# HDaoud/ORBSLAMM

Measured on AMD Instinct MI355X. Metric: frames/s ORB extract+match, 1241x376 @2000 kp; bit-exact kp/desc vs CPU, higher is better.
Workload: dtype u8

## Files before the change

### orbslamm_amd/csrc/orbx_host.inc

```

enum ProfId { P_H2D = 0, P_RESIZE, P_FAST, P_DISTRIBUTE, P_BLUR, P_ORIENT_DESC, P_MATCH_BEST2, P_MATCH_ACCEPT, P_MATCH_PRUNE, P_D2H, P_COUNT };
static const char* kProfNames[P_COUNT] = {"h2d", "k_pyramid", "k_fast", "k_distribute", "k_blur",
                                          "k_orient_desc", "k_match_mfma", "k_match_accept", "k_match_prune", "d2h"};
struct ProfSpan { int id; hipEvent_t a, b; };

struct Profiler {
    bool on = false, cur = false;
    int only = -1;
    std::vector<ProfSpan> spans;
    std::vector<hipEvent_t> pool;
    double ms[P_COUNT] = {0};
    int64_t launches[P_COUNT] = {0};
    hipEvent_t get()
    {
        if (!pool.empty()) { hipEvent_t e = pool.back(); pool.pop_back(); return e; }
        hipEvent_t e;
        (void)hipEventCreate(&e);
        return e;
    }
    void begin(int id, hipStream_t s)
    {
        cur = on && (only < 0 || only == id);
        if (!cur) return;
        ProfSpan sp{id, get(), get()};
// ... 305 lines not shown
    g.iniTh = h->prm.iniThFAST; g.minTh = h->prm.minThFAST;
    memcpy(g.umax, h->umax, sizeof g.umax);
    if (w > 8191 || h0 > 8191) return fail(ORBX_E_UNSUPPORTED, "frame larger than 8191 px");
    out.cells.clear();
    out.tabs.clear();
    int pyrOff = 0, blurOff = 0, candOff = 0, keptOff = 0, maxRoiW = 8, maxRoiH = 8, maxRoiW0 = 8, maxRoiH0 = 8, nodeCap = 16, maxCells = 1;
    for (int l = 0; l < g.nlevels; l++) {
        LevelGeom& L = g.lv[l];
        const float scale = h->mvInvScaleFactor[l];
        L.w = cv_round((double)((float)w * scale));
        L.h = cv_round((double)((float)h0 * scale));
        if (L.w < 1 || L.h < 1) return fail(ORBX_E_UNSUPPORTED, "pyramid level %d is empty", l);
        L.stride = align_up(L.w, 64);
        L.pyrOff = pyrOff;
        if (l > 0) pyrOff += align_up(L.stride * L.h, 256);
        L.blurStride = align_up(L.w, 64);
        L.blurOff = blurOff;
        blurOff += align_up(L.blurStride * L.h, 256);
        L.scale = h->mvScaleFactor[l];
        L.kpSize = (float)(int)((float)kPatchSize * h->mvScaleFactor[l]);
        L.nFeat = h->mnFeaturesPerLevel[l];

        const int minBX = kMinBorder, minBY = kMinBorder;
        const int maxBX = L.w - kEdgeThreshold + 3, maxBY = L.h - kEdgeThreshold + 3;
        L.winW = maxBX - minBX; L.winH = maxBY - minBY;
        const float W = 30;
        const float width = (float)(maxBX - minBX), height = (float)(maxBY - minBY);
        L.nCols = width > 0 ? (int)(width / W) : 0;
        L.nRows = height > 0 ? (int)(height / W) : 0;
        L.cellBase = (int)out.cells.size();
        L.nCells = 0;
        int candCap = 0;
        if (L.nCols >= 1 && L.nRows >= 1) {
            L.wCell = (int)std::ceil((double)(width / L.nCols));
            L.hCell = (int)std::ceil((double)(height / L.nRows));
            uint32_t seq = 0;
            for (int i = 0; i < L.nRows; i++) {
                const float iniY = (float)(minBY + i * L.hCell);
                float maxY = iniY + L.hCell + 6;
                if (iniY >= maxBY - 3) continue;
                if (maxY > maxBY) maxY = (float)maxBY;
                for (int j = 0; j < L.nCols; j++) {
                    const float iniX = (float)(minBX + j * L.wCell);
                    float maxX = iniX + L.wCell + 6;
                    if (iniX >= maxBX - 6) continue;
                    if (maxX > maxBX) maxX = (float)maxBX;
                    Cell c;
                    c.level = (uint16_t)l;
                    c.x0 = (uint16_t)(int)iniX; c.y0 = (uint16_t)(int)iniY;
                    c.w = (uint16_t)((int)maxX - (int)iniX); c.h = (uint16_t)((int)maxY - (int)iniY);
                    c.ci = (uint16_t)i; c.cj = (uint16_t)j;
                    c.seq = seq++;
                    c.candOff = (uint32_t)candCap;
                    if (c.w < 7 || c.h < 7) continue;
                    if (c.w > 127 || c.h > 127 || c.seq >= 65536u)
                        return fail(ORBX_E_UNSUPPORTED, "cell geometry out of range");
                    out.cells.push_back(c);
                    L.nCells++;
                    candCap += ((c.w - 6 + 1) / 2) * ((c.h - 6 + 1) / 2);
                    maxRoiW = std::max<int>(maxRoiW, c.w);
                    maxRoiH = std::max<int>(maxRoiH, c.h);
                    if (l == 0) { maxRoiW0 = std::max<int>(maxRoiW0, c.w); maxRoiH0 = std::max<int>(maxRoiH0, c.h); }
                }
            }
        }
        maxCells = std::max(maxCells, L.nCells);
        L.candOff = candOff;
        L.candCap = align_up(candCap + 8, 8);
        candOff += L.candCap;
        L.nIni = 0; L.hX = 0.f;
        if (L.winW > 0 && L.winH > 0) {
            L.nIni = (int)roundf((float)(maxBX - minBX) / (float)(maxBY - minBY));
            if (L.nIni >= 1) L.hX = (float)(maxBX - minBX) / (float)L.nIni;
            else if (L.nCells > 0)
                return fail(ORBX_E_UNSUPPORTED, "level %d: width/height < 0.5, the reference divides by zero (ORBextractor.cc:543-545)", l);
        }
        L.keptOff = keptOff;
        L.keptCap = align_up(std::max(L.nFeat + 4, 4 * L.nIni) + 4, 4);
        keptOff += L.keptCap;
        nodeCap = std::max(nodeCap, L.keptCap + 8);
    }
    g.totalCells = (int)out.cells.size();
    g.maxCellsPerLevel = maxCells;
    g.pyrFrameBytes = std::max(pyrOff, 256);
    g.blurFrameBytes = blurOff;
    g.candFrameRecs = candOff;
    g.keptFrameRecs = keptOff;
    g.maxKp = keptOff;
    out.tileStrideDw = maxRoiW + 5 <= 48 ? 12 : 20;
    if (maxRoiW + 5 > 80 || maxRoiW - 6 > 127 || maxRoiH - 6 > 127) return fail(ORBX_E_UNSUPPORTED, "cell larger than the FAST tile");
    out.tileRows = maxRoiH;
    out.fastListCap = ((maxRoiW - 6) * (maxRoiH - 6) + 63) / 64 * 64;
    out.tileRows0 = maxRoiH0;
    out.fastListCap0 = ((maxRoiW0 - 6) * (maxRoiH0 - 6) + 63) / 64 * 64;
    out.fastSmapPitch = align_up(maxRoiW - 6 + 2, 4);
    out.fastSmapPitch0 = align_up(maxRoiW0 - 6 + 2, 4);
    out.nodeCap = align_up(std::max(nodeCap, 360), 4);

    for (int l = 0; l < g.nlevels; l++) { out.xoff[l] = out.yoff[l] = 0; }
    for (int l = 1; l < g.nlevels; l++) {
        const int sw = g.lv[l - 1].w, sh = g.lv[l - 1].h, dw = g.lv[l].w, dh = g.lv[l].h;
        const double inv_scale_x = (double)dw / sw, inv_scale_y = (double)dh / sh;
        const double scale_x = 1. / inv_scale_x, scale_y = 1. / inv_scale_y;
        if (scale_x == 2.0 && scale_y == 2.0)
            return fail(ORBX_E_UNSUPPORTED, "scale factor 2: cv::resize switches to INTER_AREA (not on this path)");
        out.xoff[l] = (int)out.tabs.size();
        std::vector<short4> xt(dw);
        int xmax = dw;
        for (int dx = 0; dx < dw; dx++) {
            float fx = (float)((dx + 0.5) * scale_x - 0.5);
            int sx = (int)std::floor(fx);
            fx -= sx;
            if (sx < 0) { fx = 0; sx = 0; }
            if (sx + 1 >= sw) {
                xmax = std::min(xmax, dx);
                if (sx >= sw - 1) { fx = 0; sx = sw - 1; }
            }
            auto sat = [](float v) { long r = lrintf(v); return (short)(r > 32767 ? 32767 : (r < -32768 ? -32768 : r)); };
            xt[dx] = make_short4((short)sx, sat((1.f - fx) * 2048), sat(fx * 2048), 0);
        }
        for (int dx = 0; dx < dw; dx++) xt[dx].w = dx < xmax ? 1 : 0;
        out.tabs.insert(out.tabs.end(), xt.begin(), xt.end());
        out.yoff[l] = (int)out.tabs.size();
        for (int dy = 0; dy < dh; dy++) {
            float fy = (float)((dy + 0.5) * scale_y - 0.5);
            int sy = (int)std::floor(fy);
            fy -= sy;
            auto clip = [&](int y) { return y < 0 ? 0 : (y < sh ? y : sh - 1); };
            auto sat = [](float v) { long r = lrintf(v); return (short)(r > 32767 ? 32767 : (r < -32768 ? -32768 : r)); };
            out.tabs.push_back(make_short4((short)clip(sy), (short)clip(sy + 1), sat((1.f - fy) * 2048), sat(fy * 2048)));
        }
    }
    int tb = 0, kb = 0;
    for (int l = 0; l < g.nlevels; l++) {
        out.bt.base[l] = tb;
        out.bt.tilesX[l] = (g.lv[l].w + kBlurTW - 1) / kBlurTW;
        tb += out.bt.tilesX[l] * ((g.lv[l].h + kBlurTH - 1) / kBlurTH);
        out.kb.base[l] = kb;
        kb += (g.lv[l].keptCap + kKpPerBlock - 1) / kKpPerBlock;
    }
    for (int l = g.nlevels; l <= ORBX_MAXL; l++) { out.bt.base[l] = tb; out.kb.base[l] = kb; }
    out.blurTilesTotal = tb;
    out.kbTotal = kb;

    out.pyrFused = false;
    const int refine0 = h->maxB <= h->latMaxB ? 1 : 0;
    for (int refine = refine0; refine < 4 && !out.pyrFused; refine++) {
        const int nl = g.nlevels;
        const int top = nl - 1;
        int BX = 4 << refine, BY = 6 << refine;
        while (BX > 1 && g.lv[top].w / BX < 8) BX >>= 1;
        while (BY > 1 && g.lv[top].h / BY < 8) BY >>= 1;
        out.pyrBlocks = BX * BY;
        out.pyrRanges.assign((size_t)out.pyrBlocks * nl, PyrRange{0, 0, 0, 0, 0, 0, 0, 0});
        int maxA = 4, maxB = 4, tabCap = 4;
        for (int bj = 0; bj < BY; bj++)
            for (int bi = 0; bi < BX; bi++) {
                PyrRange* R = &out.pyrRanges[(size_t)(bj * BX + bi) * nl];
                int nx0 = 0, nx1 = 0, ny0 = 0, ny1 = 0;
                for (int l = top; l >= 0; l--) {
                    const int w = g.lv[l].w, hh = g.lv[l].h;
                    int ox0 = (int)((int64_t)bi * w / BX) & ~3, ox1 = bi + 1 == BX ? w : ((int)((int64_t)(bi + 1) * w / BX) & ~3);
                    int oy0 = (int)((int64_t)bj * hh / BY), oy1 = (int)((int64_t)(bj + 1) * hh / BY);
                    if (l == 0) ox0 = ox1 = oy0 = oy1 = 0;
                    int cx0 = ox0, cx1 = ox1, cy0 = oy0, cy1 = oy1;
                    if (l < top && nx1 > nx0 && ny1 > ny0) {
                        const short4* xt = &out.tabs[out.xoff[l + 1]];
                        const short4* yt = &out.tabs[out.yoff[l + 1]];
                        int sx0 = 1 << 30, sx1 = -1, sy0 = 1 << 30, sy1 = -1;
                        const int nx1g = std::min<int>(g.lv[l + 1].w, nx0 + ((nx1 - nx0 + 3) & ~3));
                        for (int dx = nx0; dx < nx1g; dx++) {
                            const int a = (uint16_t)xt[dx].x, b = a + (xt[dx].w ? 2 : 1);
                            sx0 = std::min(sx0, a); sx1 = std::max(sx1, b);
                        }
                        for (int dy = ny0; dy < ny1; dy++) {
                            sy0 = std::min<int>(sy0, yt[dy].x); sy1 = std::max<int>(sy1, yt[dy].y + 1);
                        }
                        sx1 = std::min(sx1, w); sy1 = std::min(sy1, hh);
                        if (cx1 > cx0 && cy1 > cy0) {
                            cx0 = std::min(cx0, sx0); cx1 = std::max(cx1, sx1);
                            cy0 = std::min(cy0, sy0); cy1 = std::max(cy1, sy1);
                        } else { cx0 = sx0; cx1 = sx1; cy0 = sy0; cy1 = sy1; }
                    }
                    cx0 &= ~3;
                    R[l] = PyrRange{(int16_t)ox0, (int16_t)ox1, (int16_t)oy0, (int16_t)oy1,
                                    (int16_t)cx0, (int16_t)cx1, (int16_t)cy0, (int16_t)cy1};
                    if (cx1 > cx0 && cy1 > cy0) {
                        const int rowBytes = (cx1 - cx0 + 3) & ~3;
                        int rows = cy1 - cy0;
                        if (l == 0 && ny1 > ny0) {
                            const short4* yt = &out.tabs[out.yoff[1]];
                            const int chh1 = ny1 - ny0;
                            rows = 0;
                            for (int sidx = 0; sidx < kPyrStrips; sidx++) {
                                const int ya = (int)((int64_t)chh1 * sidx / kPyrStrips), yb = (int)((int64_t)chh1 * (sidx + 1) / kPyrStrips);
                                if (yb > ya) rows = std::max(rows, std::min<int>(yt[ny0 + yb - 1].y + 1, cy1) - (int)yt[ny0 + ya].x);
                            }
                        }
                        const int words = rowBytes / 4 * rows + 4;
                        if (l & 1) maxB = std::max(maxB, words); else maxA = std::max(maxA, words);
                        if (l > 0) tabCap = std::max(tabCap, std::max(rowBytes, cy1 - cy0));
                    }
                    nx0 = cx0; nx1 = cx1; ny0 = cy0; ny1 = cy1;
                }
            }
        out.pyrBufA = maxA; out.pyrBufB = maxB; out.pyrTabCap = (tabCap + 3) & ~3;
        const size_t pl = ((size_t)maxA + maxB) * 4 + (size_t)out.pyrTabCap * 16;
        out.pyrFused = pl <= 64 * 1024 || (refine == 3 && pl <= 156 * 1024);
    }
    return ORBX_OK;
}

static constexpr int kMatchChunks = 4;

static size_t dist_lds_bytes(int cap, int maxCells) { return (size_t)(19 * cap + 8 + 2 * (maxCells + 1)) * 4; }

static void chain_stream_release(int device, int idx);
static void tput_streams_release(orbx_handle* h);

static void free_device(orbx_handle* h)
{
    if (h->device < 0) return;
    (void)hipSetDevice(h->device);
    if (h->stream) (void)hipStreamSynchronize(h->stream);
    for (int i = 0; i < orbx_handle::kMaxSplit; i++) {
        if (h->streamP[i]) (void)hipStreamSynchronize(h->streamP[i]);
        if (h->streamB[i]) (void)hipStreamSynchronize(h->streamB[i]);
    }
    if (h->stream3) (void)hipStreamSynchronize(h->stream3);
    h->prof.destroy();
    void* ptrs[] = {h->d_distScratch, h->d_pyrRanges, h->d_geom, h->d_cells, h->d_tabs, h->d_pyr, h->d_blur, h->d_candRaw, h->d_candA, h->d_candB,
                    h->d_candCount, h->d_cellCount, h->d_kept, h->d_keptCount, h->d_err, h->d_kps, h->d_desc, h->d_count,
                    h->d_match, h->d_binOf, h->d_hist, h->d_nmatch, h->d_partial, h->d_xdesc};
    for (void* p : ptrs) if (p) (void)hipFree(p);
    if (h->d_stereo) (void)hipFree(h->d_stereo);
    h->pool.stop();
    for (hipStream_t st : {h->streamUp, h->streamDown, h->streamUpQ, h->streamDownQ}) if (st) (void)hipStreamSynchronize(st);
    for (auto& sl : h->slot) {
        if (sl.h_in) (void)hipHostFree(sl.h_in);
        if (sl.h_out) (void)hipHostFree(sl.h_out);
        if (sl.d_in) (void)hipFree(sl.d_in);
        if (sl.d_out) (void)hipFree(sl.d_out);
        for (hipEvent_t& e : sl.evUp) if (e) (void)hipEventDestroy(e);
        if (sl.evOut) (void)hipEventDestroy(sl.evOut);
        if (sl.evPacked) (void)hipEventDestroy(sl.evPacked);
    }
    for (hipStream_t st : {h->streamUp, h->streamDown, h->streamUpQ, h->streamDownQ}) if (st) (void)hipStreamDestroy(st);
    for (int i = 0; i < orbx_handle::kMaxSplit; i++) {
        if (h->evPyr[i]) (void)hipEventDestroy(h->evPyr[i]);
        if (h->evBlur[i]) (void)hipEventDestroy(h->evBlur[i]);
        if (h->evPart[i]) (void)hipEventDestroy(h->evPart[i]);
        if (h->evFast0[i]) (void)hipEventDestroy(h->evFast0[i]);
        if (h->streamP[i] && !(i == 0 && h->chainIdx >= 0) && !h->sharedStreams) (void)hipStreamDestroy(h->streamP[i]);
        if (h->streamB[i]) (void)hipStreamDestroy(h->streamB[i]);
    }
    if (h->evStart) (void)hipEventDestroy(h->evStart);
    if (h->evDesc) (void)hipEventDestroy(h->evDesc);
    for (int i = 0; i < 2; i++) if (h->evMatch[i]) (void)hipEventDestroy(h->evMatch[i]);
    for (int i = 0; i < 2; i++) if (h->evMatched[i]) (void)hipEventDestroy(h->evMatched[i]);
    if (h->sharedStreams) tput_streams_release(h);
    if (h->stream3) (void)hipStreamDestroy(h->stream3);
    if (h->stream) (void)hipStreamDestroy(h->stream);
    if (h->chainIdx >= 0) { chain_stream_release(h->device, h->chainIdx); h->chainIdx = -1; h->streamP[0] = nullptr; }
}

struct ChainPool { hipStream_t s[4] = {nullptr, nullptr, nullptr, nullptr}; int users[4] = {0, 0, 0, 0}; bool made = false; };
static ChainPool g_chain[64];
static std::mutex g_chainMu;

static bool chain_prio_normal() { static const bool v = [] { const char* e = getenv("ORBX_LAT_PRIO"); return e && e[0] == '0'; }(); return v; }

static int chain_stream_acquire(int device, int priority, hipStream_t* out, int* idx)
{
    std::lock_guard<std::mutex> lk(g_chainMu);
    ChainPool& cp = g_chain[device & 63];
    if (!cp.made) {
        hipStream_t s[4] = {nullptr, nullptr, nullptr, nullptr};
        void* scratch = nullptr;
        hipError_t e = hipMalloc(&scratch, 256);
        for (int i = 0; i < 4 && e == hipSuccess; i++) e = hipStreamCreateWithPriority(&s[i], hipStreamNonBlocking, priority);
        for (int i = 0; i < 4 && e == hipSuccess; i++) { e = hipMemsetAsync(scratch, 0, 256, s[i]); if (e == hipSuccess) e = hipStreamSynchronize(s[i]); }
        if (scratch) (void)hipFree(scratch);
        if (e != hipSuccess) {
            for (hipStream_t st : s) if (st) (void)hipStreamDestroy(st);
            return fail(ORBX_E_HIP, "cannot make the chain streams of device %d: %s", device, hipGetErrorString(e));
        }
        for (int i = 0; i < 4; i++) cp.s[i] = s[i];
        cp.made = true;
    }
    int best = 0;
    for (int i = 1; i < 4; i++) if (cp.users[i] < cp.users[best]) best = i;
    cp.users[best]++;
    *out = cp.s[best]; *idx = best;
    return ORBX_OK;
}

static void chain_stream_release(int device, int idx)
{
    std::lock_guard<std::mutex> lk(g_chainMu);
    if (idx >= 0 && idx < 4) g_chain[device & 63].users[idx]--;
}

struct TputPool { hipStream_t host = nullptr, p[orbx_handle::kMaxSplit] = {nullptr}, match = nullptr; int users = 0; };
static TputPool g_tput[64];
static std::mutex g_tputMu;

static int tput_streams_acquire(orbx_handle* h, int device, int prHi)
{
    std::lock_guard<std::mutex> lk(g_tputMu);
    TputPool& tp = g_tput[device & 63];
    if (!tp.host) {
        TputPool t;
        void* scratch = nullptr;
        hipError_t e = hipStreamCreateWithFlags(&t.host, hipStreamNonBlocking);
        if (e == hipSuccess) e = hipStreamCreateWithPriority(&t.p[0], hipStreamNonBlocking, prHi);
        if (e == hipSuccess) e = hipStreamCreateWithPriority(&t.p[1], hipStreamNonBlocking, prHi);
        if (e == hipSuccess) e = hipStreamCreateWithFlags(&t.match, hipStreamNonBlocking);
        if (e == hipSuccess) e = hipMalloc(&scratch, 256);
        for (hipStream_t st : {t.host, t.p[0], t.p[1], t.match}) {
            if (e == hipSuccess) e = hipMemsetAsync(scratch, 0, 256, st);
            if (e == hipSuccess) e = hipStreamSynchronize(st);
        }
        if (scratch) (void)hipFree(scratch);
        for (int i = 2; i < orbx_handle::kMaxSplit && e == hipSuccess; i++) e = hipStreamCreateWithPriority(&t.p[i], hipStreamNonBlocking, prHi);
        if (e != hipSuccess) {
            for (hipStream_t st : {t.host, t.match}) if (st) (void)hipStreamDestroy(st);
            for (hipStream_t st : t.p) if (st) (void)hipStreamDestroy(st);
            return fail(ORBX_E_HIP, "cannot make the pipeline streams of device %d: %s", device, hipGetErrorString(e));
        }
        tp.host = t.host; tp.match = t.match;
        for (int i = 0; i < orbx_handle::kMaxSplit; i++) tp.p[i] = t.p[i];
    }
    tp.users++;
    h->stream = tp.host; h->stream3 = tp.match;
    for (int i = 0; i < orbx_handle::kMaxSplit; i++) h->streamP[i] = tp.p[i];
    h->sharedStreams = true;
    return ORBX_OK;
}

static void tput_streams_release(orbx_handle* h)
{
    std::lock_guard<std::mutex> lk(g_tputMu);
    TputPool& tp = g_tput[h->device & 63];
    h->stream = nullptr; h->stream3 = nullptr;
    for (int i = 0; i < orbx_handle::kMaxSplit; i++) h->streamP[i] = nullptr;
    h->sharedStreams = false;
    --tp.users;
}

static int create_handle(const OrbxParams* params, int max_w, int max_h, int max_batch, int device, int latCeil, orbx_t** out)
{
    if (!params || !out) return fail(ORBX_E_INVALID, "null argument");
    *out = nullptr;
    orbx_handle* h = new orbx_handle();
    h->latMaxB = latCeil;
    h->prm = *params;
    int rc = init_tables(h);
    if (rc) { delete h; return rc; }
    h->device = device;
    { const char* e = getenv("ORBX_SERIAL"); h->serial = e && e[0] == '1'; }
    { const char* e = getenv("ORBX_MATCH_POPCOUNT"); h->matchPopcount = e && e[0] == '1'; }
// ... 1359 lines not shown
```

### orbslamm_amd/csrc/orbx_kernels.hip

```cpp
#include <hip/hip_runtime.h>
#include <stdint.h>

#include "orbx_common.hpp"

namespace orbx {

struct FrameSrc {
    const uint8_t* img0;
    int32_t stride0;
    int64_t pitch0;
    uint8_t* pyr;
    uint8_t* blur;
    int32_t f0;
};

__device__ __forceinline__ const uint8_t* level_ptr(const Geom* g, const FrameSrc& s, int f, int l, int& stride)
{
    if (l == 0) { stride = s.stride0; return s.img0 + (int64_t)f * s.pitch0; }
    stride = g->lv[l].stride;
    return s.pyr + (int64_t)f * g->pyrFrameBytes + g->lv[l].pyrOff;
}

__device__ __forceinline__ bool xcd_block_frame(int nframes, int& blk, int& fr)
{
    if (nframes < 8) { blk = blockIdx.x; fr = blockIdx.y; return true; }
    const int total = gridDim.x;
    const int lin = blockIdx.y * total + blockIdx.x;
    const int k = lin >> 3;
    fr = (k / total) * 8 + (lin & 7);
    blk = k - (k / total) * total;
    return fr < nframes;
}

__device__ __forceinline__ uint64_t lanemask_lt()
{
    const uint32_t lane = threadIdx.x & 63;
    return lane == 0 ? 0ull : (~0ull >> (64 - lane));
}

struct ResizeTabs {
    const short4* xtab[ORBX_MAXL];
    const short4* ytab[ORBX_MAXL];
};

__global__ __launch_bounds__(256) void k_resize_level(const Geom* __restrict__ g, FrameSrc src, ResizeTabs tabs, int level)
{
    const int lw = g->lv[level].w, lh = g->lv[level].h, dstStride = g->lv[level].stride;
    const int f = blockIdx.z + src.f0;
    const int x4 = (blockIdx.x * 64 + threadIdx.x) * 4;
    const int dy = blockIdx.y * 4 + threadIdx.y;
    if (x4 >= lw || dy >= lh) return;
    int sstride;
    const uint8_t* S = level_ptr(g, src, f, level - 1, sstride);
    uint8_t* D = src.pyr + (int64_t)f * g->pyrFrameBytes + g->lv[level].pyrOff + (int64_t)dy * dstStride;
    const short4 yt = tabs.ytab[level][dy];
    const uint8_t* S0 = S + (int64_t)yt.x * sstride;
    const uint8_t* S1 = S + (int64_t)yt.y * sstride;
    const int b0 = yt.z, b1 = yt.w;
    uint32_t packed = 0;
#pragma unroll
    for (int i = 0; i < 4; i++) {
        const short4 xt = tabs.xtab[level][min(x4 + i, lw - 1)];
        const int sx = (uint16_t)xt.x;
        int r0, r1;
        if (xt.w) {
            r0 = S0[sx] * xt.y + S0[sx + 1] * xt.z;
            r1 = S1[sx] * xt.y + S1[sx + 1] * xt.z;
        } else {
            r0 = S0[sx] * 2048;
            r1 = S1[sx] * 2048;
        }
        const int v = (((b0 * (r0 >> 4)) >> 16) + ((b1 * (r1 >> 4)) >> 16) + 2) >> 2;
        packed |= (uint32_t)(v & 0xFF) << (8 * i);
    }
    *(uint32_t*)(D + x4) = packed;
}

constexpr int kPyrStrips = 2;
#ifndef ORBX_DESC_PRIO
#define ORBX_DESC_PRIO 0
#endif
#ifndef ORBX_BLUR_PRIO
#define ORBX_BLUR_PRIO 0
#endif
#ifndef ORBX_DIST_PRIO
#define ORBX_DIST_PRIO 0
#endif
#ifndef ORBX_PYR_PRIO
#define ORBX_PYR_PRIO 3
#endif
#ifndef ORBX_PYR_THREADS
#define ORBX_PYR_THREADS 256
#endif
constexpr int kPyrThreads = ORBX_PYR_THREADS;
struct PyrRange {
    int16_t ox0, ox1, oy0, oy1;
    int16_t nx0, nx1, ny0, ny1;
};

__global__ __launch_bounds__(kPyrThreads) void k_pyramid(const Geom* __restrict__ g, FrameSrc src, ResizeTabs tabs,
                                                const PyrRange* __restrict__ ranges, int bufAWords, int bufBWords,
                                                int tabCap, int xcdFrames)
{
    extern __shared__ __attribute__((aligned(16))) uint32_t plds[];
#if ORBX_PYR_PRIO
    __builtin_amdgcn_s_setprio(ORBX_PYR_PRIO);
#endif
    uint8_t* const ldsb = (uint8_t*)plds;
    const int offBuf[2] = {0, bufAWords * 4};
    uint2* const sxt = (uint2*)(plds + bufAWords + bufBWords);
    uint2* const syt = sxt + tabCap;
    int pblk = (int)blockIdx.x, pfr = (int)blockIdx.y;
    if (xcdFrames >= 8 && !xcd_block_frame(xcdFrames, pblk, pfr)) return;
    const int f = pfr + src.f0;
    const int nl = g->nlevels;
    const PyrRange* R = ranges + (int64_t)pblk * nl;
    const int tid = threadIdx.x;

    PyrRange p = R[0];
    int pstride = 0;
    const bool have0 = p.nx1 > p.nx0 && p.ny1 > p.ny0;
    int stride0 = 0;
    const uint8_t* S0 = nullptr;
    int ndw0 = 0;
    if (have0) {
        const uint8_t* S = level_ptr(g, src, f, 0, stride0);
        ndw0 = (p.nx1 - p.nx0 + 3) >> 2;
        pstride = ndw0 * 4;
        S0 = S + p.nx0;
    }
    constexpr int T = kPyrThreads;
    constexpr int kStripRegs = 4096 / T;
    uint32_t sreg[kStripRegs];
    auto strip_rows = [&](int strip, int chh1, const uint2* yt, int& r0, int& r1) {
        const int ya = (int)((int64_t)chh1 * strip / kPyrStrips), yb = (int)((int64_t)chh1 * (strip + 1) / kPyrStrips);
        r0 = r1 = 0;
        if (yb > ya) { r0 = (int16_t)(yt[ya].x & 0xFFFF); r1 = min((int)(int16_t)(yt[yb - 1].x >> 16) + 1, (int)p.ny1); }
    };
    const int q256 = have0 ? T / ndw0 : 0, m256 = have0 ? T - q256 * ndw0 : 0;
    const int rowT = have0 ? tid / ndw0 : 0, colT = have0 ? tid - rowT * ndw0 : 0;
    auto fetch0 = [&](int r0, int r1) {
        const int total = (r1 - r0) * ndw0;
        if (total <= 0 || total > T * kStripRegs) return;
        const uint8_t* Sr = S0 + (int64_t)r0 * stride0;
        int r = rowT, c = colT;
#pragma unroll
        for (int k = 0; k < kStripRegs; k++) {
            if (k * T < total) {
                if (k * T + tid < total) sreg[k] = *(const uint32_t*)(Sr + (int64_t)r * stride0 + 4 * c);
                r += q256; c += m256;
                if (c >= ndw0) { c -= ndw0; r++; }
            }
        }
    };
    auto commit0 = [&](int r0, int r1) {
        const int total = (r1 - r0) * ndw0;
        if (total <= 0) return;
        if (total <= T * kStripRegs) {
#pragma unroll
            for (int k = 0; k < kStripRegs; k++) {
                const int i = k * T + tid;
                if (i < total) plds[i] = sreg[k];
            }
            return;
        }
        const uint8_t* Sr = S0 + (int64_t)r0 * stride0;
        for (int i0 = 0; i0 < total; i0 += T * 8) {
            uint32_t regs[8];
#pragma unroll
            for (int k = 0; k < 8; k++) {
                const int i = min(i0 + k * T + tid, total - 1);
                const int r = i / ndw0, c = i - r * ndw0;
                regs[k] = *(const uint32_t*)(Sr + (int64_t)r * stride0 + 4 * c);
            }
#pragma unroll
            for (int k = 0; k < 8; k++) {
                const int i = i0 + k * T + tid;
                if (i < total) plds[i] = regs[k];
            }
        }
    };
    for (int l = 1; l < nl; l++) {
        const PyrRange c = R[l];
        const int cw = c.nx1 - c.nx0, chh = c.ny1 - c.ny0;
        const int gpr = (cw + 3) >> 2;
        const int cstride = gpr * 4;
        const int lw = g->lv[l].w, dstStride = g->lv[l].stride;
        uint8_t* const D = src.pyr + (int64_t)f * g->pyrFrameBytes + g->lv[l].pyrOff;
        const int pnx0 = p.nx0, pny0 = p.ny0;
        const uint2* __restrict__ gx_tab = (const uint2*)tabs.xtab[l];
        const uint2* __restrict__ gy_tab = (const uint2*)tabs.ytab[l];
        for (int i = tid; i < cstride; i += T) sxt[i] = gx_tab[min(c.nx0 + i, lw - 1)];
        for (int i = tid; i < chh; i += T) syt[i] = gy_tab[c.ny0 + i];
        __syncthreads();
        const int offP = offBuf[(l - 1) & 1], offC = offBuf[l & 1];
        const bool strips = l == 1 && have0 && chh > 0;
        const int nstrips = strips ? kPyrStrips : 1;
        if (strips) { int r0, r1; strip_rows(0, chh, syt, r0, r1); fetch0(r0, r1); }
        for (int strip = 0; strip < nstrips; strip++) {
        const int ya = strips ? (int)((int64_t)chh * strip / nstrips) : 0, yb = strips ? (int)((int64_t)chh * (strip + 1) / nstrips) : chh;
        int prow0 = pny0;
        if (strips) {
            int r0, r1;
            strip_rows(strip, chh, syt, r0, r1);
            prow0 = r0;
            if (strip) __syncthreads();
            commit0(r0, r1);
            __syncthreads();
            if (strip + 1 < nstrips) { int q0, q1; strip_rows(strip + 1, chh, syt, q0, q1); fetch0(q0, q1); }
        }
        if (gpr > 0 && yb > ya) {
          for (int gxb = 0; gxb < gpr; gxb += T) {
            const int cols = min(T, gpr - gxb);
            const int dr = T / cols;
            const int yy0 = tid / cols, gx = gxb + tid - yy0 * cols;
            if (yy0 < dr) {
                int sx[4], a0[4], a1[4];
#pragma unroll
                for (int i = 0; i < 4; i++) {
                    const uint2 xt = sxt[4 * gx + i];
                    sx[i] = (int)(xt.x & 0xFFFF) - pnx0;
                    a0[i] = (int16_t)(xt.x >> 16);
                    a1[i] = (int16_t)(xt.y & 0xFFFF);
                }
                const int dx = c.nx0 + 4 * gx;
                const bool ownX = dx >= c.ox0 && dx < c.ox1;
                for (int yy = ya + yy0; yy < yb; yy += dr) {
                    const uint2 yt = syt[yy];
                    const int sy0 = (int16_t)(yt.x & 0xFFFF), sy1 = (int16_t)(yt.x >> 16);
                    const int b0 = (int16_t)(yt.y & 0xFFFF), b1 = (int16_t)(yt.y >> 16);
                    const int o0 = offP + (sy0 - prow0) * pstride;
                    const int o1 = offP + (sy1 - prow0) * pstride;
                    uint32_t packed = 0;
#pragma unroll
                    for (int i = 0; i < 4; i++) {
                        const int s00 = ldsb[o0 + sx[i]], s10 = ldsb[o1 + sx[i]];
                        const int r0 = s00 * a0[i] + ldsb[o0 + sx[i] + 1] * a1[i];
                        const int r1 = s10 * a0[i] + ldsb[o1 + sx[i] + 1] * a1[i];
                        const int v = (((b0 * (r0 >> 4)) >> 16) + ((b1 * (r1 >> 4)) >> 16) + 2) >> 2;
                        packed |= (uint32_t)(v & 0xFF) << (8 * i);
                    }
                    plds[(offC >> 2) + yy * gpr + gx] = packed;
                    const int dy = c.ny0 + yy;
                    if (ownX && dy >= c.oy0 && dy < c.oy1)
                        *(uint32_t*)(D + (int64_t)dy * dstStride + dx) = packed;
                }
            }
          }
        }
        }
        p = c;
        pstride = cstride;
        __syncthreads();
    }
}

__device__ __forceinline__ int min3i(int a, int b, int c) { return min(min(a, b), c); }
__device__ __forceinline__ int max3i(int a, int b, int c) { return max(max(a, b), c); }

template <int TSB, int K> struct RingOff {
    static constexpr int cx[16] = {0, 1, 2, 3, 3, 3, 2, 1, 0, -1, -2, -3, -3, -3, -2, -1};
    static constexpr int cy[16] = {3, 3, 2, 1, 0, -1, -2, -3, -3, -3, -2, -1, 0, 1, 2, 3};
    static constexpr int v = cx[K] + cy[K] * TSB;
};

__device__ __forceinline__ int arc_max_of_min(const int (&d)[16])
{
    int m3[16], m9[16];
#pragma unroll
    for (int k = 0; k < 16; k++) m3[k] = min3i(d[k], d[(k + 1) & 15], d[(k + 2) & 15]);
#pragma unroll
    for (int k = 0; k < 16; k++) m9[k] = min3i(m3[k], m3[(k + 3) & 15], m3[(k + 6) & 15]);
    int a5[5];
#pragma unroll
    for (int k = 0; k < 5; k++) a5[k] = max3i(m9[3 * k], m9[3 * k + 1], m9[3 * k + 2]);
    return max(max3i(a5[0], a5[1], a5[2]), max3i(a5[3], a5[4], m9[15]));
}

template <int TSB> __device__ __forceinline__ void ring_load(const uint8_t* __restrict__ p, int (&r)[16])
{
    r[0] = p[RingOff<TSB, 0>::v];   r[1] = p[RingOff<TSB, 1>::v];   r[2] = p[RingOff<TSB, 2>::v];   r[3] = p[RingOff<TSB, 3>::v];
    r[4] = p[RingOff<TSB, 4>::v];   r[5] = p[RingOff<TSB, 5>::v];   r[6] = p[RingOff<TSB, 6>::v];   r[7] = p[RingOff<TSB, 7>::v];
    r[8] = p[RingOff<TSB, 8>::v];   r[9] = p[RingOff<TSB, 9>::v];   r[10] = p[RingOff<TSB, 10>::v]; r[11] = p[RingOff<TSB, 11>::v];
    r[12] = p[RingOff<TSB, 12>::v]; r[13] = p[RingOff<TSB, 13>::v]; r[14] = p[RingOff<TSB, 14>::v]; r[15] = p[RingOff<TSB, 15>::v];
}

template <int SW> __device__ __forceinline__ uint32_t pk_min3(uint32_t a, uint32_t b, uint32_t c)
{
    uint32_t r;
    if (SW == 0) asm("v_pk_minimum3_f16 %0, %1, %2, %3" : "=v"(r) : "v"(a), "v"(b), "v"(c));
    else if (SW == 4) asm("v_pk_minimum3_f16 %0, %1, %2, %3 op_sel:[0,0,1] op_sel_hi:[1,1,0]" : "=v"(r) : "v"(a), "v"(b), "v"(c));
    else if (SW == 6) asm("v_pk_minimum3_f16 %0, %1, %2, %3 op_sel:[0,1,1] op_sel_hi:[1,0,0]" : "=v"(r) : "v"(a), "v"(b), "v"(c));
    else asm("v_pk_minimum3_f16 %0, %1, %2, %3 op_sel:[0,1,0] op_sel_hi:[1,0,1]" : "=v"(r) : "v"(a), "v"(b), "v"(c));
    static_assert(SW == 0 || SW == 2 || SW == 4 || SW == 6, "exchange masks in use");
    return r;
}
template <int SW> __device__ __forceinline__ uint32_t pk_max3(uint32_t a, uint32_t b, uint32_t c)
{
    uint32_t r;
    if (SW == 0) asm("v_pk_maximum3_f16 %0, %1, %2, %3" : "=v"(r) : "v"(a), "v"(b), "v"(c));
    else if (SW == 4) asm("v_pk_maximum3_f16 %0, %1, %2, %3 op_sel:[0,0,1] op_sel_hi:[1,1,0]" : "=v"(r) : "v"(a), "v"(b), "v"(c));
    else if (SW == 6) asm("v_pk_maximum3_f16 %0, %1, %2, %3 op_sel:[0,1,1] op_sel_hi:[1,0,0]" : "=v"(r) : "v"(a), "v"(b), "v"(c));
    else asm("v_pk_maximum3_f16 %0, %1, %2, %3 op_sel:[0,1,0] op_sel_hi:[1,0,1]" : "=v"(r) : "v"(a), "v"(b), "v"(c));
    static_assert(SW == 0 || SW == 2 || SW == 4 || SW == 6, "exchange masks in use");
    return r;
}
template <bool MAXMIN> __device__ __forceinline__ int arc_fold_pk(const int (&r)[16])
{
    uint32_t X[8], M3[8], M9[8];
#pragma unroll
    for (int k = 0; k < 8; k++) X[k] = (uint32_t)r[k] | ((uint32_t)r[k + 8] << 16);
#define ORBX_IN(SW, a, b, c) (MAXMIN ? pk_min3<SW>(a, b, c) : pk_max3<SW>(a, b, c))
#define ORBX_OUT(SW, a, b, c) (MAXMIN ? pk_max3<SW>(a, b, c) : pk_min3<SW>(a, b, c))
#pragma unroll
    for (int k = 0; k < 6; k++) M3[k] = ORBX_IN(0, X[k], X[k + 1], X[k + 2]);
    M3[6] = ORBX_IN(4, X[6], X[7], X[0]);
    M3[7] = ORBX_IN(6, X[7], X[0], X[1]);
    M9[0] = ORBX_IN(0, M3[0], M3[3], M3[6]);
    M9[1] = ORBX_IN(0, M3[1], M3[4], M3[7]);
    M9[2] = ORBX_IN(4, M3[2], M3[5], M3[0]);
    M9[3] = ORBX_IN(4, M3[3], M3[6], M3[1]);
    M9[4] = ORBX_IN(4, M3[4], M3[7], M3[2]);
    M9[5] = ORBX_IN(6, M3[5], M3[0], M3[3]);
    M9[6] = ORBX_IN(6, M3[6], M3[1], M3[4]);
    M9[7] = ORBX_IN(6, M3[7], M3[2], M3[5]);
    const uint32_t A = ORBX_OUT(0, M9[0], M9[1], M9[2]);
    const uint32_t B = ORBX_OUT(0, M9[3], M9[4], M9[5]);
    const uint32_t C = ORBX_OUT(0, M9[6], M9[7], A);
    const uint32_t D = ORBX_OUT(4, B, C, B);
    const uint32_t E = ORBX_OUT(2, D, C, D);
#undef ORBX_IN
#undef ORBX_OUT
    return (int)(E & 0xFFFFu);
}

template <int TSB> __device__ __forceinline__ int fast_S_dark(const uint8_t* __restrict__ p)
{
    int r[16];
    ring_load<TSB>(p, r);
    return max((int)p[0] - arc_fold_pk<false>(r), 0);
}
template <int TSB> __device__ __forceinline__ int fast_S_bright(const uint8_t* __restrict__ p)
{
    int r[16];
    ring_load<TSB>(p, r);
    return max(arc_fold_pk<true>(r) - (int)p[0], 0);
}

template <int TSB> __device__ __forceinline__ int fast_S(const uint8_t* __restrict__ p)
{
    int r[16], d[16];
    ring_load<TSB>(p, r);
    const int v = p[0];
#pragma unroll
    for (int k = 0; k < 16; k++) d[k] = v - r[k];
    const int A = arc_max_of_min(d);
#pragma unroll
    for (int k = 0; k < 16; k++) d[k] = -d[k];
    return max(max(A, arc_max_of_min(d)), 0);
}

__device__ __forceinline__ uint64_t ballot64(bool b) { return __builtin_amdgcn_ballot_w64(b); }
__device__ __forceinline__ uint64_t tail_mask(int n) { return n >= 64 ? ~0ull : (1ull << n) - 1; }
__device__ __forceinline__ int lanes_below(uint64_t bal)
{
    return __builtin_amdgcn_mbcnt_hi((uint32_t)(bal >> 32), __builtin_amdgcn_mbcnt_lo((uint32_t)bal, 0));
}

#ifdef ORBX_FAST_STATS
__device__ unsigned long long g_fastStats[16];
#endif
template <int TSB>
__global__ __launch_bounds__(64) void k_fast(const Geom* __restrict__ g, const Cell* __restrict__ cells,
                                            FrameSrc src, uint64_t* __restrict__ cand,
                                            int32_t* __restrict__ cellCount, int32_t* __restrict__ errFlag,
                                            int tileRows, int listCap, int smapPitch, int nframes, int cell0)
{
    extern __shared__ __attribute__((aligned(16))) uint32_t lds[];
    constexpr int TSD = TSB / 4;
    int bx, fr;
    if (!xcd_block_frame(nframes, bx, fr)) return;
    bx += cell0;
    const Cell c = cells[bx];
    const int f = fr + src.f0;
    const int lane = threadIdx.x;
    const int level = c.level;
    const LevelGeom& L = g->lv[level];
    int stride;
    const uint8_t* base = level_ptr(g, src, f, level, stride);

#ifdef ORBX_FAST_STATS
    unsigned long long tk0 = wall_clock64(), tk1;
    const bool statCell = lane == 0 && (blockIdx.x & 63) == 0;
#define FAST_TICK(i) do { tk1 = wall_clock64(); if (statCell) atomicAdd(&g_fastStats[i], tk1 - tk0); tk0 = tk1; } while (0)
#else
#define FAST_TICK(i) do { } while (0)
#endif
    uint32_t* tile = lds;
// ... 1493 lines not shown
```

Measured before the change: 184,100.

## Tune pyramid resize inner loop: precomputed LDS offsets, chunk widths, packed rounding

The y-table now stores row offsets relative to the previous-level LDS buffer, computed once per strip, so the inner loop does not recompute them per output row. The host picks a per-strip column chunk width that minimises wavefront-iterations, replacing the fixed width of T. Ownership tests move to a single unsigned range compare with incrementally stepped pointers. Rounding and packing use SDWA inline assembly plus v_perm. The fused-pyramid condition also gains a per-buffer size cap. This adds ISA-specific asm and a bigger PyrRange struct, and bit-exactness depends on the packed adds never overflowing their 16-bit halves.

```diff
diff --git a/orbslamm_amd/csrc/orbx_host.inc b/orbslamm_amd/csrc/orbx_host.inc
--- a/orbslamm_amd/csrc/orbx_host.inc
+++ b/orbslamm_amd/csrc/orbx_host.inc
@@ -481,7 +481,7 @@
         while (BX > 1 && g.lv[top].w / BX < 8) BX >>= 1;
         while (BY > 1 && g.lv[top].h / BY < 8) BY >>= 1;
         out.pyrBlocks = BX * BY;
-        out.pyrRanges.assign((size_t)out.pyrBlocks * nl, PyrRange{0, 0, 0, 0, 0, 0, 0, 0});
+        out.pyrRanges.assign((size_t)out.pyrBlocks * nl, PyrRange{0, 0, 0, 0, 0, 0, 0, 0, {}});
         int maxA = 4, maxB = 4, tabCap = 4;
         for (int bj = 0; bj < BY; bj++)
             for (int bi = 0; bi < BX; bi++) {
@@ -513,7 +513,14 @@
                     }
                     cx0 &= ~3;
                     R[l] = PyrRange{(int16_t)ox0, (int16_t)ox1, (int16_t)oy0, (int16_t)oy1,
-                                    (int16_t)cx0, (int16_t)cx1, (int16_t)cy0, (int16_t)cy1};
+                                    (int16_t)cx0, (int16_t)cx1, (int16_t)cy0, (int16_t)cy1, {}};
+                    if (l > 0 && cx1 > cx0 && cy1 > cy0) {
+                        const int gpr = (cx1 - cx0 + 3) >> 2, rows = cy1 - cy0;
+                        for (int sidx = 0; sidx < kPyrStrips; sidx++) {
+                            const int ya = (int)((int64_t)rows * sidx / kPyrStrips), yb = (int)((int64_t)rows * (sidx + 1) / kPyrStrips);
+                            R[l].cw[sidx] = (int16_t)pyr_chunk_width(gpr, l == 1 ? yb - ya : rows, kPyrThreads);
+                        }
+                    }
                     if (cx1 > cx0 && cy1 > cy0) {
                         const int rowBytes = (cx1 - cx0 + 3) & ~3;
                         int rows = cy1 - cy0;
@@ -535,7 +542,7 @@
             }
         out.pyrBufA = maxA; out.pyrBufB = maxB; out.pyrTabCap = (tabCap + 3) & ~3;
         const size_t pl = ((size_t)maxA + maxB) * 4 + (size_t)out.pyrTabCap * 16;
-        out.pyrFused = pl <= 64 * 1024 || (refine == 3 && pl <= 156 * 1024);
+        out.pyrFused = pl <= 64 * 1024 || (refine == 3 && pl <= 156 * 1024 && std::max(maxA, maxB) <= 16 * 1024);
     }
     return ORBX_OK;
 }
diff --git a/orbslamm_amd/csrc/orbx_kernels.hip b/orbslamm_amd/csrc/orbx_kernels.hip
--- a/orbslamm_amd/csrc/orbx_kernels.hip
+++ b/orbslamm_amd/csrc/orbx_kernels.hip
@@ -93,10 +93,41 @@
 #define ORBX_PYR_THREADS 256
 #endif
 constexpr int kPyrThreads = ORBX_PYR_THREADS;
-struct PyrRange {
+struct alignas(4) PyrRange {
     int16_t ox0, ox1, oy0, oy1;
     int16_t nx0, nx1, ny0, ny1;
+    int16_t cw[kPyrStrips];
 };
+
+static inline int pyr_chunk_cost(int gpr, int rows, int c, int T)
+{
+    int cost = 0;
+    for (int g0 = 0; g0 < gpr; g0 += c) {
+        const int cols = gpr - g0 < c ? gpr - g0 : c, dr = T / cols;
+        cost += (cols * dr + 63) / 64 * ((rows + dr - 1) / dr);
+    }
+    return cost;
+}
+static inline int pyr_chunk_width(int gpr, int rows, int T)
+{
+    if (gpr <= 0 || rows <= 0) return 1;
+    int best = gpr < T ? gpr : T, bestCost = pyr_chunk_cost(gpr, rows, best, T);
+    for (int c = best - 1; c >= 1; c--) {
+        const int cost = pyr_chunk_cost(gpr, rows, c, T);
+        if (cost < bestCost) { best = c; bestCost = cost; }
+    }
+    return best;
+}
+
+__device__ __forceinline__ uint32_t pyr_round_pack(uint32_t sum0, uint32_t q01, uint32_t q11, uint32_t sum2, uint32_t q03, uint32_t q13)
+{
+    asm("v_add_u32_sdwa %0, %2, %3 dst_sel:WORD_1 dst_unused:UNUSED_PRESERVE src0_sel:WORD_1 src1_sel:WORD_1\n\t"
+        "v_add_u32_sdwa %1, %4, %5 dst_sel:WORD_1 dst_unused:UNUSED_PRESERVE src0_sel:WORD_1 src1_sel:WORD_1\n\t"
+        "v_add_u32_e32 %0, 0x20002, %0\n\t"
+        "v_add_u32_e32 %1, 0x20002, %1"
+        : "+v"(sum0), "+v"(sum2) : "v"(q01), "v"(q11), "v"(q03), "v"(q13));
+    return __builtin_amdgcn_perm(sum2 >> 2, sum0 >> 2, 0x06040200u);
+}
 
 __global__ __launch_bounds__(kPyrThreads) void k_pyramid(const Geom* __restrict__ g, FrameSrc src, ResizeTabs tabs,
                                                 const PyrRange* __restrict__ ranges, int bufAWords, int bufBWords,
@@ -132,10 +163,10 @@
     constexpr int T = kPyrThreads;
     constexpr int kStripRegs = 4096 / T;
     uint32_t sreg[kStripRegs];
-    auto strip_rows = [&](int strip, int chh1, const uint2* yt, int& r0, int& r1) {
+    auto strip_rows = [&](int strip, int chh1, const short4* __restrict__ yt, int& r0, int& r1) {
         const int ya = (int)((int64_t)chh1 * strip / kPyrStrips), yb = (int)((int64_t)chh1 * (strip + 1) / kPyrStrips);
         r0 = r1 = 0;
-        if (yb > ya) { r0 = (int16_t)(yt[ya].x & 0xFFFF); r1 = min((int)(int16_t)(yt[yb - 1].x >> 16) + 1, (int)p.ny1); }
+        if (yb > ya) { r0 = yt[ya].x; r1 = min((int)yt[yb - 1].y + 1, (int)p.ny1); }
     };
     const int q256 = have0 ? T / ndw0 : 0, m256 = have0 ? T - q256 * ndw0 : 0;
     const int rowT = have0 ? tid / ndw0 : 0, colT = have0 ? tid - rowT * ndw0 : 0;
@@ -189,61 +220,86 @@
         uint8_t* const D = src.pyr + (int64_t)f * g->pyrFrameBytes + g->lv[l].pyrOff;
         const int pnx0 = p.nx0, pny0 = p.ny0;
         const uint2* __restrict__ gx_tab = (const uint2*)tabs.xtab[l];
-        const uint2* __restrict__ gy_tab = (const uint2*)tabs.ytab[l];
+        const uint2* __restrict__ gy_tab = (const uint2*)tabs.ytab[l] + c.ny0;
+        const short4* __restrict__ gy_rows = tabs.ytab[l] + c.ny0;
+        const bool strips = l == 1 && have0 && chh > 0;
+        const int nstrips = strips ? kPyrStrips : 1;
+        int srow0[kPyrStrips];
+#pragma unroll
+        for (int s = 0; s < kPyrStrips; s++) {
+            srow0[s] = pny0;
+            if (strips) { int r1; strip_rows(s, chh, gy_rows, srow0[s], r1); }
+        }
+        if (strips) { int r0, r1; strip_rows(0, chh, gy_rows, r0, r1); fetch0(r0, r1); }
         for (int i = tid; i < cstride; i += T) sxt[i] = gx_tab[min(c.nx0 + i, lw - 1)];
-        for (int i = tid; i < chh; i += T) syt[i] = gy_tab[c.ny0 + i];
+        for (int i = tid; i < chh; i += T) {
+            const uint2 yt = gy_tab[i];
+            int prow = srow0[0];
+#pragma unroll
+            for (int s = 1; s < kPyrStrips; s++)
+                if (strips && i >= (int)((int64_t)chh * s / kPyrStrips)) prow = srow0[s];
+            const uint32_t o0 = (uint32_t)(((int)(int16_t)(yt.x & 0xFFFF) - prow) * pstride);
+            const uint32_t o1 = (uint32_t)(((int)(int16_t)(yt.x >> 16) - prow) * pstride);
+            syt[i] = make_uint2((o0 & 0xFFFF) | (o1 << 16), yt.y);
+        }
         __syncthreads();
         const int offP = offBuf[(l - 1) & 1], offC = offBuf[l & 1];
-        const bool strips = l == 1 && have0 && chh > 0;
-        const int nstrips = strips ? kPyrStrips : 1;
-        if (strips) { int r0, r1; strip_rows(0, chh, syt, r0, r1); fetch0(r0, r1); }
         for (int strip = 0; strip < nstrips; strip++) {
         const int ya = strips ? (int)((int64_t)chh * strip / nstrips) : 0, yb = strips ? (int)((int64_t)chh * (strip + 1) / nstrips) : chh;
-        int prow0 = pny0;
         if (strips) {
             int r0, r1;
-            strip_rows(strip, chh, syt, r0, r1);
-            prow0 = r0;
+            strip_rows(strip, chh, gy_rows, r0, r1);
             if (strip) __syncthreads();
             commit0(r0, r1);
             __syncthreads();
-            if (strip + 1 < nstrips) { int q0, q1; strip_rows(strip + 1, chh, syt, q0, q1); fetch0(q0, q1); }
+            if (strip + 1 < nstrips) { int q0, q1; strip_rows(strip + 1, chh, gy_rows, q0, q1); fetch0(q0, q1); }
         }
         if (gpr > 0 && yb > ya) {
-          for (int gxb = 0; gxb < gpr; gxb += T) {
-            const int cols = min(T, gpr - gxb);
+          int C = c.cw[0];
+#pragma unroll
+          for (int s = 1; s < kPyrStrips; s++) if (strip == s) C = c.cw[s];
+          C = min(max(C, 1), T);
+          for (int gxb = 0; gxb < gpr; gxb += C) {
+            const int cols = min(C, gpr - gxb);
             const int dr = T / cols;
             const int yy0 = tid / cols, gx = gxb + tid - yy0 * cols;
             if (yy0 < dr) {
-                int sx[4], a0[4], a1[4];
+                uint32_t sxo[4], a0[4], a1[4];
 #pragma unroll
                 for (int i = 0; i < 4; i++) {
                     const uint2 xt = sxt[4 * gx + i];
-                    sx[i] = (int)(xt.x & 0xFFFF) - pnx0;
-                    a0[i] = (int16_t)(xt.x >> 16);
-                    a1[i] = (int16_t)(xt.y & 0xFFFF);
+                    sxo[i] = (uint32_t)(offP + (int)(xt.x & 0xFFFF) - pnx0);
+                    a0[i] = xt.x >> 16;
+                    a1[i] = xt.y & 0xFFFF;
                 }
                 const int dx = c.nx0 + 4 * gx;
                 const bool ownX = dx >= c.ox0 && dx < c.ox1;
-                for (int yy = ya + yy0; yy < yb; yy += dr) {
-                    const uint2 yt = syt[yy];
-                    const int sy0 = (int16_t)(yt.x & 0xFFFF), sy1 = (int16_t)(yt.x >> 16);
-                    const int b0 = (int16_t)(yt.y & 0xFFFF), b1 = (int16_t)(yt.y >> 16);
-                    const int o0 = offP + (sy0 - prow0) * pstride;
-                    const int o1 = offP + (sy1 - prow0) * pstride;
-                    uint32_t packed = 0;
+                const int ownA = ownX ? min(max(ya, c.oy0 - c.ny0), yb) : yb;
+                const int ownB = ownX ? max(ownA, min(yb, c.oy1 - c.ny0)) : yb;
+                const uint32_t nOwn = (uint32_t)(ownB - ownA);
+                const int tEnd = yb - ownA;
+                const int y0 = ya + yy0;
+                const uint2* yp = syt + y0;
+                uint32_t* outp = plds + (offC >> 2) + y0 * gpr + gx;
+                uint32_t goff = (uint32_t)((c.ny0 + y0) * dstStride + dx);
+                const uint32_t gstep = (uint32_t)(dr * dstStride);
+                for (int t = y0 - ownA; t < tEnd; t += dr, yp += dr, outp += dr * gpr, goff += gstep) {
+                    const uint2 yt = *yp;
+                    const uint32_t o0 = yt.x & 0xFFFF, o1 = yt.x >> 16;
+                    const uint32_t b0 = yt.y & 0xFFFF, b1 = yt.y >> 16;
+                    uint32_t q0[4], q1[4];
 #pragma unroll
                     for (int i = 0; i < 4; i++) {
-                        const int s00 = ldsb[o0 + sx[i]], s10 = ldsb[o1 + sx[i]];
-                        const int r0 = s00 * a0[i] + ldsb[o0 + sx[i] + 1] * a1[i];
-                        const int r1 = s10 * a0[i] + ldsb[o1 + sx[i] + 1] * a1[i];
-                        const int v = (((b0 * (r0 >> 4)) >> 16) + ((b1 * (r1 >> 4)) >> 16) + 2) >> 2;
-                        packed |= (uint32_t)(v & 0xFF) << (8 * i);
+                        const uint32_t p0 = sxo[i] + o0, p1 = sxo[i] + o1;
+                        const uint32_t s00 = ldsb[p0], s10 = ldsb[p1];
+                        const uint32_t r0 = s00 * a0[i] + ldsb[p0 + 1] * a1[i];
+                        const uint32_t r1 = s10 * a0[i] + ldsb[p1 + 1] * a1[i];
+                        q0[i] = b0 * (r0 >> 4);
+                        q1[i] = b1 * (r1 >> 4);
                     }
-                    plds[(offC >> 2) + yy * gpr + gx] = packed;
-                    const int dy = c.ny0 + yy;
-                    if (ownX && dy >= c.oy0 && dy < c.oy1)
-                        *(uint32_t*)(D + (int64_t)dy * dstStride + dx) = packed;
+                    const uint32_t packed = pyr_round_pack((q0[0] >> 16) + (q1[0] >> 16), q0[1], q1[1], (q0[2] >> 16) + (q1[2] >> 16), q0[3], q1[3]);
+                    *outp = packed;
+                    if ((uint32_t)t < nOwn) *(uint32_t*)(D + goff) = packed;
                 }
             }
           }
```

New measurement: 185,000 (median of 6 runs). Within noise of the previous version (+0.5%).
